# tonfengerqiguyisui/mapping-private

Hardware: AMD Instinct MI355X
Metric: Mvoxels/s C3-HLAC + detections/s sliding-box, 256^3 grid (higher is better)
Workload: dtype u8 x u8 -> u32 (exact integer C3-HLAC), f32 search

## Files before the change

mapping-private_amd/csrc/c3h_internal.h:

```cpp
#pragma once
#include <hip/hip_runtime.h>

#include <cstdint>
#include <cstdlib>
#include <string>
#include <mutex>
#include <vector>

#include "../../include/c3hlac_mi355x.h"

namespace c3h {

constexpr uint32_t kOcc = 1u << 24;
constexpr uint32_t kEmptyKey = 0xffffffffu;
constexpr int kBlock = 256;
constexpr int kTileMax = 16;

constexpr float kNorm0 = 1 / 255.0;
constexpr float kNorm1 = 1 / 65025.0;
constexpr float kNorm117_1 = 1 / 845325.0;
constexpr float kNorm117_1Bin = 1 / 13.0;

template <class T>
struct DevBuf {
  T* p = nullptr;
  size_t n = 0;
};

struct SearchLists {
  int rank = 0, M = 0;
  std::vector<double> score;
  std::vector<int32_t> x, y, z, mode;
// ... 207 lines not shown
  int atomic;
  const uint32_t* lut;
  float* feat;
  int32_t* exist;
  unsigned long long* acc64;
  const int16_t* axmap;
  int ar_s = 0, ar_oy = 0, ar_oz = 0;
  uint32_t ar_magic = 0;
  int32_t* work;
  int32_t* rows;
  uint32_t epoch;
  int zero_empty;
  int zero_feat;
  int64_t ntiles;
  long long* prof;
  int debug;
  uint32_t* dense = nullptr;
  _Float16* feat16 = nullptr;
  uint32_t* feat16_flag = nullptr;
  int f16s = 0;
  const uint32_t* vl_words = nullptr;
  const int32_t* vl_counts = nullptr;
  int vl_nseg = 0, vl_seg = 0, vl_count_stride = 0;
};

int64_t c3hlac_grid(const C3Launch& a);
hipError_t launch_c3hlac(const C3Launch& a, hipStream_t s);
hipError_t launch_colour_hist(const uint32_t* grid, int64_t nvox, unsigned long long* out, hipStream_t s);
hipError_t launch_offcell_delta(const int32_t* rec, int nrec, const C3Launch& l, int hist1, const int off[3],
                                const int sb[3], float inv_s, hipStream_t s);
hipError_t launch_c3_finalize(const unsigned long long* acc64, int64_t hist_num, int variant,
                              float* feat, int32_t* exist, int nframes, hipStream_t s);
struct NbrGrid {
  const float4* pts;
  int64_t n;
  float origin[3];
  float cell, inv_cell;
  int dim[3];
  const uint32_t* sorted;
  const uint32_t* cstart;
  const uint32_t* cend;
};
struct GrsdArgs {
  const float4* cent;
  int64_t nc;
  const int32_t* layout;
// ... 117 lines not shown
};
hipError_t launch_replay(const double* scores, const ReplayModes& modes, int M, int rank,
                         int r1, int r2, int r3, int clean, c3h_det* lists, c3h_det* out2,
                         hipStream_t s);
struct ReplayFrames {
  const double* scores;
  int64_t s_scores;
  ReplayModes modes;
  int M, nf, rank;
  int r1, r2, r3;
  int clean;
  c3h_det* lists;
  int64_t s_lists;
  c3h_det* outs[kMaxBatch];
};
bool replay_frames_ok(const ReplayModes& modes, int rank);
hipError_t launch_replay_frames(const ReplayFrames& a, hipStream_t s);

hipError_t launch_clean_lists(c3h_det* lists, int n, hipStream_t s);

struct TickParts {
  const C3Launch* occ = nullptr;
  const C3Launch* tile = nullptr;
  const SparseSearch* gate = nullptr;
  const SparseCompress* comp = nullptr;
  const SparseSearch* score = nullptr;
  DevBuf<long long>* prof = nullptr;
};
bool tick_ok(const C3Launch& l);
hipError_t launch_tick(const TickParts& p, hipStream_t s);
size_t c3hlac_lds_bytes(int tw_max, int list_max);
int64_t leaf_layout_blocks(int64_t nvox);

}

struct c3h_ctx {
  int device = 0;
  hipStream_t stream = nullptr;
  hipStream_t own_stream = nullptr;
  std::string err;

  c3h_ctx* parent = nullptr;
  std::vector<c3h_ctx*> lanes;
  std::vector<hipEvent_t> lane_ev;
  hipEvent_t fork_ev = nullptr;
  int nlanes = 3;
// ... 37 lines not shown
  bool vcent_valid = false;
  int64_t n_offcell = 0;
  c3h::DevBuf<uint32_t> scratch;
  c3h::DevBuf<uint32_t> tmp_u32;
  c3h::DevBuf<int32_t> tmp_i32;
  uint32_t* h_small = nullptr;
  c3h::VoxFrameRec* h_recs = nullptr;
  size_t h_recs_n = 0;
  bool table_valid = false;

  bool have_feat = false;
  c3h_extract_params last{};
  int64_t hist_num = 0;
  int32_t subdiv_b[3] = {0, 0, 0};
  int feat_dim = 0;
  c3h::DevBuf<float> feat;
  c3h::DevBuf<int32_t> exist;
  c3h::DevBuf<unsigned long long> acc64;
  c3h::DevBuf<int32_t> segs;
  c3h::DevBuf<int16_t> axmap;
  std::vector<int16_t> h_axmap;
  c3h::DevBuf<uint32_t> tileflags;
  c3h::DevBuf<int32_t> work;
  uint32_t tile_epoch = 0;
  int cap_h2d = 0;
  int64_t tf_stride = -1;
  int tf_frames = 0;
  int nframes_feat = 1;
  c3h::DevBuf<int32_t> rows;
  bool rows_valid = false;
  bool g_sparse = false;
  bool feat_sparse = false;
  c3h::DevBuf<long long> glist;
  c3h::DevBuf<float> gbox;
  c3h::DevBuf<uint32_t> gcnt;
  uint32_t search_epoch = 0;
  int gcnt_frames = 0;
  c3h::DevBuf<long long> prof;
  c3h::DevBuf<unsigned long long> chist;

  std::vector<int32_t> h_segs;
  c3h::DevBuf<uint32_t> lut;
  bool lut_ready = false;

  bool have_setup = false;
  int D = 0, F = 0, M = 0, r = 0, Dpad = 0;
// ... 31 lines not shown
  size_t h_dl_n = 0;
  c3h::DevBuf<c3h_det> d_lists;
  bool lists_host_valid = true;
  bool lists_dev_valid = false;
  int32_t last_range[3] = {0, 0, 0};

  c3h::Timer timer;

  bool capture = false;
  bool cap_c3_valid = false, cap_search_valid = false, cap_sparse_g = false, cap_argmax = false;
  c3h::C3Launch cap_c3{};
  c3h::SparseSearch cap_q{};
  c3h::SparseCompress cap_sc{};
  bool cap_replay = false;
  c3h::ReplayFrames cap_rp{};

  struct PipeBatch {
    c3h::C3Launch l;
    c3h::SparseSearch q;
    c3h::SparseCompress sc;
    int nf;
    int age;
    bool stamped = false;
    c3h_ctx* set = nullptr;
    std::vector<int64_t> layout;
    bool fix = false;
    c3h::PointFixup fx{};
    bool replay = false;
    c3h::ReplayFrames rp{};
  };
  struct PipeKey {
    int32_t div_b[3], min_b[3];
    float leaf;
    c3h_extract_params p;
    int32_t range[3], thr, rotate, batch, rank;
    uint64_t setup_version;
  };
  c3h::DevBuf<uint32_t> pb_grid, pb_wlist;
  c3h::DevBuf<int32_t> pb_part, pb_lim;
  c3h::DevBuf<c3h::VoxFlag> pb_flags;
  c3h::DevBuf<uint32_t> pb_bucket, pb_xcnt;
  c3h::DevBuf<uint32_t> dense_flag;
  c3h::DevBuf<c3h::VoxMoved> pb_moved;
  int64_t pb_cvox = 0;
  int pb_slots = 0;
  int pb_prev_nf = 0, pb_prev_total = 0;
// ... 20 lines not shown
```

mapping-private_amd/csrc/c3hlac_dev.h:

```cpp
#pragma once
#include <type_traits>

#include "c3h_internal.h"
#include "occ_sched.h"

namespace c3h {

constexpr int kArrStride = 196;
constexpr int kChunk = 128;
constexpr int kGroups = kChunk / 4;

__device__ __forceinline__ int bin981(int k, int c, int n) {
  return k <= 8 ? 6 + 78 * c + 9 * n + k : 60 + 78 * c + 4 * n + (k - 9);
}
__device__ __forceinline__ int tri6(int c, int n) { return 6 * c - c * (c - 1) / 2 + (n - c); }

__device__ __forceinline__ int bin_of(int type, int k, int n, int c) {
  if (k <= 12) return (type ? 495 : 0) + bin981(k, c, n);
  if (k == 13) {
    if (type == 0) return c <= n ? 474 + tri6(c, n) : -1;
    if (c <= 1 && n >= 2) return 969 + 4 * c + (n - 2);
    if ((c == 2 || c == 3) && n >= 4) return 977 + 2 * (c - 2) + (n - 4);
    return -1;
  }
// ... 63 lines not shown
    if (cur == -1) {
      const int old = atomicCAS(&s_set[h], -1, t);
      if (old == -1 || old == t) return;
    }
  }
  stamp_tile(t, epoch, flags, cnt, work);
}

struct OccArgs {
  const uint32_t* grid[kMaxBatch];
  int gx, gy, gz;
  const int16_t* axmap;
  int ns0, ns1;
  int ntiles;
  uint32_t epoch;
  uint32_t* tf;
  int32_t* work;
  int64_t s_tf, s_work;
  int contiguous;
  int steal_from = 0, steal_unit = 0, steal_units = 0, nframes = 0, steal_wgs = 0;
  int ar_s = 0, ar_oy = 0, ar_oz = 0;
  uint32_t ar_magic = 0;
  const uint32_t* dense = nullptr;
};

constexpr int kOccBitsMax = 1 << 18;
#ifndef C3H_OCC_PIPE
#define C3H_OCC_PIPE 0
#endif
#ifndef C3H_OCC_ARITH
#define C3H_OCC_ARITH 1
#endif
constexpr bool kOccArith = C3H_OCC_ARITH;
#ifndef C3H_OCC_PAIR
#define C3H_OCC_PAIR 1
#endif
#ifndef C3H_OCC_RING
#define C3H_OCC_RING 0
#endif
static_assert(kOccSchedBlock == kBlock, "occ_sched.h: threads per streaming workgroup");
constexpr bool kOccPipe = C3H_OCC_PIPE;
typedef unsigned int v4u __attribute__((ext_vector_type(4)));
constexpr int kAxLds = 3072;

__device__ __forceinline__ int block_excl_scan(int v, int* s_wsum, int* total) {
  const int lane = threadIdx.x & 63, wid = threadIdx.x >> 6;
// ... 112 lines not shown
    uint32_t mA = 0, mB = 0;
    bool cplx = false;
#pragma unroll
    for (int k = 0; k < 4; ++k) {
      if (tx0[k] < 0) continue;
      if (tA < 0 || tx0[k] == tA) {
        tA = tx0[k];
        mA |= 1u << k;
      } else if (tB < 0 || tx0[k] == tB) {
        tB = tx0[k];
        mB |= 1u << k;
      } else {
        cplx = true;
      }
    }
    const bool pair_ok = C3H_OCC_PAIR && __ballot(cplx) == 0ull;
    constexpr int kRow = kOccRowUnroll;
    constexpr int kChunkR = kBlock * kRow;
    const int lg = gx == 256 ? 8 : gx == 512 ? 9 : 10;
    const OccSched sc =
        occ_sched(n4, kRow, gdx, oa.contiguous, oa.steal_from, oa.steal_unit, oa.steal_units, oa.nframes);
    const int64_t nch = sc.nch, nstat = sc.nstat;
    uint4 w[kRow];
    auto chunk_of = [&](int64_t i) { return occ_chunk_of(sc, bx, i); };
    auto load_row = [&](uint64_t base, uint32_t voff, int j) {
      uint64_t bj = base + (uint64_t)j * (kBlock * 16);
      asm volatile("" : "+s"(bj));
      typedef const __attribute__((address_space(1))) char* gptr;
      const v4u t = __builtin_nontemporal_load(
          reinterpret_cast<const __attribute__((address_space(1))) v4u*>(reinterpret_cast<gptr>(bj) + voff));
      return make_uint4(t.x, t.y, t.z, t.w);
    };
    auto chunk_base = [&](int64_t c, uint32_t& voff) {
      uint64_t base = reinterpret_cast<uint64_t>(g4) + (uint64_t)c * (kChunkR * 16);
      voff = (uint32_t)tid * 16u;
      asm volatile("" : "+s"(base), "+v"(voff));
      return base;
    };
    auto load_any = [&](int64_t c) {
      uint32_t voff;
      if (occ_chunk_whole(sc, c)) {
        const uint64_t base = chunk_base(c, voff);
#pragma unroll
        for (int j = 0; j < kRow; ++j) w[j] = load_row(base, voff, j);
      } else {
        const uint64_t base = chunk_base(c, voff);
#pragma unroll
        for (int j = 0; j < kRow; ++j)
          w[j] = occ_wave_load_inside(sc, c, j, wv) ? load_row(base, voff, j) : make_uint4(0, 0, 0, 0);
      }
    };
    auto proc = [&](uint32_t row0) {
      int y = (int)(row0 % (uint32_t)gy), z = (int)(row0 / (uint32_t)gy);
#pragma unroll
      for (int j = 0; j < kRow; ++j) {
        const int yj = y, zjj = z;
        y += rpj;
        while (y >= gy) {
          y -= gy;
          ++z;
        }
        const uint32_t ws[4] = {w[j].x, w[j].y, w[j].z, w[j].w};
        if (__ballot((ws[0] | ws[1] | ws[2] | ws[3]) != 0u) == 0ull || zjj >= gz) continue;
        int a, b;
        if (oa.ar_s) {
          a = yj >= oa.ar_oy ? (int)__umulhi((uint32_t)(yj - oa.ar_oy), oa.ar_magic) : -1;
          b = zjj >= oa.ar_oz ? (int)__umulhi((uint32_t)(zjj - oa.ar_oz), oa.ar_magic) : -1;
        } else {
          a = __builtin_amdgcn_readfirstlane(my[yj]);
          b = __builtin_amdgcn_readfirstlane(mz[zjj]);
        }
        if (a < 0 || b < 0) continue;
        const int tyz = ns0 * (a + ns1 * b);
        if (pair_ok) {
          const uint32_t o = min(ws[0], 1u) | (min(ws[1], 1u) << 1) | (min(ws[2], 1u) << 2) | (min(ws[3], 1u) << 3);
          const int ta = tA + tyz, tb = tB + tyz;
          if (o & mA) atomicOr(&s_bits[ta >> 5], 1u << (ta & 31));
          if (o & mB) atomicOr(&s_bits[tb >> 5], 1u << (tb & 31));
          continue;
        }
#pragma unroll
        for (int k = 0; k < 4; ++k) {
          const int t = tx0[k] + tyz;
          if (ws[k] && tx0[k] >= 0 && t != last) {
            last = t;
            atomicOr(&s_bits[t >> 5], 1u << (t & 31));
          }
        }
      }
    };
#if C3H_OCC_RING
    const int64_t nfull = min(n4 / kChunkR, nstat);
    int64_t ri = 0;
    if (chunk_of(0) < nfull) {
#if C3H_OCC_RING == 2
      auto chunk_rsrc = [&](int64_t c) { return reinterpret_cast<const char*>(g4 + c * kChunkR); };
      auto ring_load = [&](const char* r, int j) {
        return __builtin_nontemporal_load(reinterpret_cast<const v4u*>(r + voff + j * kBlock * 16));
      };
#else
      auto chunk_rsrc = [&](int64_t c) {
        return __builtin_amdgcn_make_buffer_rsrc((void*)(g4 + c * kChunkR), (short)0, kChunkR * 16, 0x00020000);
      };
      auto ring_load = [&](__amdgpu_buffer_rsrc_t r, int j) {
        return __builtin_amdgcn_raw_buffer_load_b128(r, voff, j * kBlock * 16, 2);
      };
#endif
      int64_t cur = chunk_of(0);
      {
        const auto r = chunk_rsrc(cur);
#pragma unroll
        for (int j = 0; j < kRow; ++j) {
// ... 54 lines not shown
    if (kOccPipe && chunk_of(0) < nch) load_chunk(w, chunk_of(0) * kChunkR);
    for (int64_t i = 0; i < sc.per; ++i) {
#endif
      const int64_t cidx = chunk_of(i);
      if (cidx >= nstat) continue;
      const int64_t c0 = cidx * kChunkR;
      uint4 nx[kRow];
      if constexpr (kOccPipe) {
        const int64_t cn = chunk_of(i + 1);
        if (cn < nch) load_chunk(nx, cn * kChunkR);
      } else {
        load_any(cidx);
      }
      const uint32_t row0 = (uint32_t)(((uint64_t)c0 * 4 + (uint64_t)wv * 256) >> lg);
#ifdef C3H_OCC_NOPROC
      {
        uint32_t o = 0;
#pragma unroll
        for (int j = 0; j < kRow; ++j) o |= w[j].x | w[j].y | w[j].z | w[j].w;
        if (o == 0x12345678u) atomicOr(&s_bits[0], 1u);
        continue;
      }
#endif
      proc(row0);
      if constexpr (kOccPipe) {
#pragma unroll
        for (int j = 0; j < kRow; ++j) w[j] = nx[j];
      }
    }
    __syncthreads();
    occ_flush_bits(s_bits, nwords, s_list, s_wsum, epoch, flags, cnt, work);
    if (oa.steal_unit > 0) {
      uint32_t* pool = oa.tf;
      for (;;) {
        __syncthreads();
        if (tid == 0) s_wsum[15] = (int)atomicAdd(pool, 1u);
        __syncthreads();
        const int u = __builtin_amdgcn_readfirstlane(s_wsum[15]);
        if (u >= oa.steal_units) {
          if (tid == 0 && atomicAdd(oa.tf + 1, 1u) == (uint32_t)oa.steal_wgs - 1) {
            atomicExch(pool, 0u);
            atomicExch(oa.tf + 1, 0u);
          }
          break;
        }
        const OccUnit un = occ_unit(sc, u);
        const int fu = un.frame;
        for (int i = tid; i < nwords; i += kBlock) s_bits[i] = 0u;
        last = -1;
        g4 = reinterpret_cast<const uint4*>(oa.grid[fu]);
        __syncthreads();
        for (int64_t c = un.cb; c < un.ce; ++c) {
          load_any(c);
          proc((uint32_t)(((uint64_t)c * kChunkR * 4 + (uint64_t)wv * 256) >> lg));
        }
        __syncthreads();
        occ_flush_bits(s_bits, nwords, s_list, s_wsum, epoch, oa.tf + fu * oa.s_tf + 4,
                       oa.tf + fu * oa.s_tf + 2 + (epoch & 1), oa.work + fu * oa.s_work);
      }
    }
    return;
  }
  uint4 w[kOccBitsUnroll];
  int64_t c0 = bx * (int64_t)kChunk4;
  if (c0 < n4) load_chunk(w, c0);
  for (; c0 < n4; c0 += cstride) {
    uint4 nx[kOccBitsUnroll];
    if (kOccPipe && c0 + cstride < n4) load_chunk(nx, c0 + cstride);
    const uint32_t v0 = (uint32_t)((c0 + tid) << 2);
    const uint32_t row0 = v0 / (uint32_t)gx;
    int x = (int)(v0 - row0 * (uint32_t)gx);
    int y = (int)(row0 % (uint32_t)gy), z = (int)(row0 / (uint32_t)gy);
    int tyz[kOccBitsUnroll];
    int txj[kOccBitsUnroll];
#pragma unroll
    for (int j = 0; j < kOccBitsUnroll; ++j) {
      const int ty = my[y], tz = mz[min(z, gz - 1)];
// ... 65 lines not shown
  int tw_max, list_max;
  int thr_r, thr_g, thr_b;
  int variant, atomic;
  const uint32_t* lut;
  float* feat;
  int32_t* exist;
  unsigned long long* acc64;
  const uint32_t* flags;
  const int32_t* work;
  uint32_t* workcnt;
  int32_t* rows;
  uint32_t epoch;
  int ntiles;
  int zero_feat;
  int zblocks;
  long long* prof;
  int wave117;
  int mfma;
  int mf_pb;
  _Float16* feat16;
  uint32_t* feat16_flag;
  int f16s;
  int debug;
};

constexpr int kMaxLoads = 4;
constexpr int kSegLds = 64;
#ifndef C3H_TILE_PREFETCH
#define C3H_TILE_PREFETCH 0
#endif
static __device__ const uint4 kHaloZero16 = {0u, 0u, 0u, 0u};

struct HaloGeo {
  int y0, z0, ly, TY, q4, n, xs;
  bool vec;
};
__device__ __forceinline__ HaloGeo halo_geo(const KArgs& a, const int32_t* segs, int tile);

#define C3H_PROF(k, cond) \
  if (fprof && tid == 0 && (cond)) fprof[bx * 8 + (k)] = (long long)wall_clock64()

__device__ __forceinline__ HaloGeo halo_geo(const KArgs& a, const int32_t* segs, int tile) {
  const int ix = tile % a.ns0, iy = (tile / a.ns0) % a.ns1, iz = tile / (a.ns0 * a.ns1);
  const int32_t* sx = segs + 3 * ix;
  const int32_t* sy = segs + 3 * (a.seg_stride + iy);
  const int32_t* sz = segs + 3 * (2 * a.seg_stride + iz);
// ... 363 lines not shown
      float* row = ffeat + (int64_t)tj * a.variant;
      for (int c = lane; c < a.variant; c += 64) row[c] = 0.0f;
      if (lane == 0) fexist[tj] = 0;
    }
  }
}

struct W117Geom {
  int x0, lx, y0, ly, z0, lz;
  int64_t h;
};

__device__ __forceinline__ W117Geom w117_geom(const KArgs& a, const int32_t* segs, int tile) {
  const int ix = tile % a.ns0, iy = (tile / a.ns0) % a.ns1, iz = tile / (a.ns0 * a.ns1);
  const int32_t* sx = segs + 3 * ix;
  const int32_t* sy = segs + 3 * (a.seg_stride + iy);
  const int32_t* sz = segs + 3 * (2 * a.seg_stride + iz);
  W117Geom g;
  g.x0 = sx[0]; g.lx = sx[1]; g.y0 = sy[0]; g.ly = sy[1]; g.z0 = sz[0]; g.lz = sz[1];
  g.h = sx[2] + (int64_t)sy[2] * a.sbx + (int64_t)sz[2] * a.sbx * a.sby;
  return g;
}

__device__ __forceinline__ void w117_load_halo(const KArgs& a, const uint32_t* __restrict__ fgrid, const W117Geom& g,
                                               bool valid, int lane, uint32_t (&hv)[kW117HaloRegs]) {
  const int TX = g.lx + 2, TY = g.ly + 2, n = valid ? TX * TY * (g.lz + 1) : 0;
  int q = lane / TX, r = lane - (lane / TX) * TX;
  const int sq = 64 / TX, sr = 64 - sq * TX;
#pragma unroll
  for (int j = 0; j < kW117HaloRegs; ++j) {
    const int e = lane + 64 * j;
    const int yy = g.y0 - 1 + q % TY, zz = g.z0 - 1 + q / TY, xx = g.x0 - 1 + r;
    const bool in = e < n && (unsigned)xx < (unsigned)a.gx && (unsigned)yy < (unsigned)a.gy &&
                    (unsigned)zz < (unsigned)a.gz;
    const uint32_t v = fgrid[in ? ((int64_t)zz * a.gy + yy) * a.gx + xx : 0];
    hv[j] = in ? v : 0u;
    q += sq;
    r += sr;
    if (r >= TX) {
      r -= TX;
      ++q;
    }
  }
}

__device__ __forceinline__ void wave_lds_fence() { __asm__ volatile("s_waitcnt lgkmcnt(0)" ::: "memory"); }

typedef unsigned short w117_u16x2 __attribute__((ext_vector_type(2)));

__device__ __forceinline__ uint32_t w117_pk(uint32_t l) { return (l & 0xffu) | ((l & 0xff00u) << 8); }
__device__ __forceinline__ uint32_t w117_beta(bool bt) { return bt ? 1u : 0x10000u; }

__device__ __forceinline__ uint32_t udot2(uint32_t x, uint32_t y, uint32_t acc) {
  return __builtin_amdgcn_udot2(__builtin_bit_cast(w117_u16x2, x), __builtin_bit_cast(w117_u16x2, y), acc, false);
}

__device__ __forceinline__ void c3hlac_wave117_body(const KArgs& a, int bx, int fy_, int gdx, uint32_t* smem) {
  const int64_t fy = fy_;
// ... 20 lines not shown
  uint16_t* s_list = reinterpret_cast<uint16_t*>(s_halo + ((a.tw_max + 3) & ~3));
  uint32_t* s_ch = s_halo + ((a.tw_max + 3) & ~3) + (((a.list_max + 1) / 2 + 3) & ~3);
  uint16_t* s_ch16 = reinterpret_cast<uint16_t*>(s_ch);
  const int NW = (gdx - a.zblocks) * kW117Waves;
  int wi = (bx - a.zblocks) * kW117Waves + wave;
  int t_cur = wi < a.ntiles ? fwork[wi] : 0;
  int t_nxt = wi + NW < a.ntiles ? fwork[wi + NW] : 0;
  const int nwork = (int)fworkcnt[a.epoch & 1];
  s_lut[tid] = a.lut[tid];
  const bool segs_lds = a.seg_stride <= kSegLds;
  const int32_t* segs = segs_lds ? s_segs : a.segs;
  if (segs_lds)
    for (int e = tid; e < 9 * a.seg_stride; e += kBlock) s_segs[e] = a.segs[e];
  lds_barrier();
  C3H_PROF(1, true);
  if (wave >= kW117Waves || wi >= nwork) return;
  bool first = true;
  int X0, Y0, X1 = 0, Y1 = 0;
  w117_bin_channels(lane, X0, Y0);
  const bool has1 = lane + 64 < 117;
  if (has1) w117_bin_channels(lane + 64, X1, Y1);
  uint32_t hv[kW117HaloRegs];
  W117Geom g = w117_geom(a, segs, t_cur);
  w117_load_halo(a, fgrid, g, true, lane, hv);
  const int thr_r = a.thr_r, thr_g = a.thr_g, thr_b = a.thr_b;
  for (; wi < nwork; wi += NW) {
    const int TX = g.lx + 2, TY = g.ly + 2, TXY = TX * TY;
    const int nh = TXY * (g.lz + 1);
    int nlist = 0;
    {
      int q = lane / TX, r = lane - q * TX;
      int qy = q % TY, qz = q / TY;
      const int sq = 64 / TX, sr = 64 - sq * TX;
#pragma unroll
      for (int j = 0; j < kW117HaloRegs; ++j) {
        const int e = lane + 64 * j;
        if (e < nh) s_halo[e] = hv[j];
        const bool occ = e < nh && hv[j] != 0u && (unsigned)(r - 1) < (unsigned)g.lx &&
                         (unsigned)(qy - 1) < (unsigned)g.ly && qz >= 1;
        const unsigned long long m = __ballot(occ);
        if (occ) s_list[nlist + __popcll(m & ((1ull << lane) - 1))] = (uint16_t)e;
        nlist += __popcll(m);
        r += sr;
        qy += sq;
        if (r >= TX) {
          r -= TX;
          ++qy;
        }
        while (qy >= TY) {
          qy -= TY;
          ++qz;
        }
      }
    }
    const W117Geom gc = g;
    const bool more = wi + NW < nwork;
    const int t_after = wi + 2 * NW < a.ntiles ? fwork[wi + 2 * NW] : 0;
    if (more) {
      g = w117_geom(a, segs, t_nxt);
      w117_load_halo(a, fgrid, g, true, lane, hv);
    }
    t_nxt = t_after;
    wave_lds_fence();
    C3H_PROF(2, first);
    C3H_PROF(3, first);
    uint32_t acc0 = 0, acc1 = 0;
    for (int c0 = 0; c0 < nlist; c0 += 64) {
      uint32_t one = 0, cA[3] = {0, 0, 0}, cB[3] = {0, 0, 0}, cN[3] = {0, 0, 0}, cQ[3] = {0, 0, 0};
      if (c0 + lane < nlist) {
        const int ti = s_list[c0 + lane];
        uint32_t wn[13];
#pragma unroll
        for (int k = 0; k < 13; ++k) {
          const int rdx = k <= 8 ? k / 3 - 1 : (k <= 11 ? k - 10 : -1);
          const int rdy = k <= 8 ? k % 3 - 1 : (k <= 11 ? -1 : 0);
          const int rdz = k <= 8 ? -1 : 0;
          wn[k] = s_halo[ti + rdx + rdy * TX + rdz * TXY];
        }
        const uint32_t w = s_halo[ti];
        const uint32_t r = (w >> 16) & 0xffu, gg = (w >> 8) & 0xffu, b = w & 0xffu;
        one = 1;
        cA[0] = w117_pk(s_lut[r]);
        cA[1] = w117_pk(s_lut[gg]);
        cA[2] = w117_pk(s_lut[b]);
        cB[0] = w117_beta((int)r > thr_r);
// ... 88 lines not shown
```

mapping-private_amd/csrc/capi.hip:

```cpp
#include <algorithm>
#include <climits>
#include <cmath>
#include <cstdio>
#include <cstdlib>
#include <cstring>
#include <thread>

#include "c3h_internal.h"

using c3h::DevBuf;

namespace {

int fail(c3h_ctx* ctx, int code, const std::string& msg) {
  if (ctx) ctx->err = msg;
  return code;
}
int hip_fail(c3h_ctx* ctx, const char* what, hipError_t e) {
  return fail(ctx, C3H_ERR_HIP, std::string(what) + ": " + hipGetErrorString(e));
}

#define HIPCHK(expr)                                     \
  do {                                                   \
    hipError_t e_ = (expr);                              \
    if (e_ != hipSuccess) return hip_fail(ctx, #expr, e_); \
  } while (0)

template <class T>
int ensure(c3h_ctx* ctx, DevBuf<T>& b, size_t n) {
  if (n == 0) n = 1;
  if (b.n >= n) return C3H_OK;
// ... 684 lines not shown
  release(ctx->vosch_feat);
  release(ctx->vacc);
  release(ctx->vmg);
  release(ctx->vtpos);
  release(ctx->vlcnt);
  release(ctx->vlists);
  release(ctx->vcnt);
  release(ctx->vpart);
  release(ctx->vcounts);
  release(ctx->voffs);
  release(ctx->vcur);
  release(ctx->vbucket);
  release(ctx->vcent);
  release(ctx->voffcell);
  release(ctx->scratch);
  release(ctx->tmp_u32);
  release(ctx->tmp_i32);
  release(ctx->feat);
  release(ctx->exist);
  release(ctx->acc64);
  release(ctx->segs);
  release(ctx->axmap);
  release(ctx->tileflags);
  release(ctx->rows);
  release(ctx->work);
  release(ctx->glist);
  release(ctx->gbox);
  release(ctx->gcnt);
  release(ctx->lut);
  release(ctx->axis_pt);
  release(ctx->axis_pt16);
  release(ctx->axis_q);
  release(ctx->fmax);
  release(ctx->G);
  release(ctx->scores);
  release(ctx->qt);
  release(ctx->partials);
  release(ctx->d_lists);
  release(ctx->prof);
  release(ctx->chist);
  release(ctx->qt16);
  release(ctx->pb_grid);
  release(ctx->pb_wlist);
  release(ctx->pb_part);
  release(ctx->pb_lim);
  release(ctx->dense_flag);
// ... 663 lines not shown
        return -1;
      };
      const int oy = first(my, div[1]), oz = first(mz, div[2]);
      int S = 0;
      if (oy >= 0) {
        while (oy + S < div[1] && my[oy + S] == 0) ++S;
      }
      const uint32_t magic = S > 0 ? (uint32_t)(0x100000000ull / (uint64_t)S) + 1u : 0u;
      auto closed = [&](const int16_t* m, int n, int off) {
        if (off < 0) return false;
        for (int c = 0; c < n; ++c) {
          const int v = c >= off ? (int)(((uint64_t)(uint32_t)(c - off) * magic) >> 32) : -1;
          if (v != m[c]) return false;
        }
        return true;
      };
      const bool ok = S > 0 && oz >= 0 && closed(my, div[1], oy) && closed(mz, div[2], oz);
      l.ar_s = ok ? S : 0;
      l.ar_oy = oy;
      l.ar_oz = oz;
      l.ar_magic = magic;
    }
    ENSURE(ctx->work, (size_t)nf * ntiles);
    l.tf = ctx->tileflags.p;
    l.work = ctx->work.p;
    l.rows = nullptr;
    if (!atomic) {
      ENSURE(ctx->rows, (size_t)nf * hist_num);
      l.rows = ctx->rows.p;
    }
    ctx->rows_valid = !atomic;
    l.epoch = ctx->tile_epoch;
    l.zero_empty = (!atomic && all_covered) ? 1 : 0;
    l.zero_feat = 0;
    ctx->feat_sparse = l.zero_empty && !l.zero_feat;
    l.ntiles = ntiles;
    l.debug = 0;
    l.prof = nullptr;
    l.dense = nullptr;
    const bool from_list = kVoxListStamp && !ctx->capture && nf == 1 && ctx->table_valid &&
                           ctx->grid_ptr == ctx->grid.p && ctx->vargs.lists &&
                           (int64_t)ctx->vns * 16 < (int64_t)div[0] * div[1] * div[2];
    if (from_list) {
      const c3h::VoxArgs& va = ctx->vargs;
      l.vl_words = va.lists + (size_t)(2 + va.par) * va.lcap;
      l.vl_counts = va.part + (size_t)va.par * va.nblk_cap * c3h::vox_part_words() + c3h::kVoxPartNew;
// ... 652 lines not shown
}

struct PipeScope {
  c3h_ctx* ctx;
  hipStream_t saved[kPipeDepth - 1];
  explicit PipeScope(c3h_ctx* c) : ctx(c) {
    ctx->pipe_busy = true;
    for (int l = 0; l < kPipeDepth - 1 && l < (int)ctx->lanes.size(); ++l) {
      saved[l] = ctx->lanes[l]->stream;
      ctx->lanes[l]->stream = ctx->stream;
    }
  }
  ~PipeScope() {
    for (int l = 0; l < kPipeDepth - 1 && l < (int)ctx->lanes.size(); ++l) ctx->lanes[l]->stream = saved[l];
    ctx->pipe_busy = false;
  }
};

int pipe_tick(c3h_ctx* ctx, const c3h_ctx::PipeBatch* fresh) {
  c3h::TickParts tp;
  tp.prof = &ctx->prof;
  if (fresh && !fresh->stamped) tp.occ = &fresh->l;
  for (auto& b : ctx->pipe) {
    if (b.age == 1) tp.tile = &b.l;
    if (b.age == 2) {
      tp.gate = &b.q;
      tp.comp = &b.sc;
    }
    if (b.age == 3) tp.score = &b.q;
  }
  {
    Timed tm(ctx, 5, fresh ? fresh->nf : 0);
    hipError_t e = c3h::launch_tick(tp, ctx->stream);
    if (e != hipSuccess) return hip_fail(ctx, "launch_tick", e);
  }
  for (auto& b : ctx->pipe) {
    if (b.age == 3 && b.replay) {
      Timed tm(ctx, 4, b.nf);
      hipError_t e = c3h::launch_replay_frames(b.rp, ctx->stream);
      if (e != hipSuccess) return hip_fail(ctx, "launch_replay_frames", e);
    }
    if (b.age == 2 && b.set) b.set->scores_layout = b.layout;
    if (b.age == 1 && b.fix) {
      hipError_t e = c3h::launch_point_fixup(b.fx, ctx->stream);
      if (e != hipSuccess) return hip_fail(ctx, "launch_point_fixup", e);
    }
  }
  std::vector<c3h_ctx::PipeBatch> next;
  for (auto& b : ctx->pipe)
    if (b.age < 3) {
      next.push_back(b);
      next.back().age++;
    }
  if (fresh) {
    next.push_back(*fresh);
    next.back().age = 1;
  }
  ctx->pipe.swap(next);
  return C3H_OK;
}

int pipe_flush(c3h_ctx* ctx) {
  if (ctx->pipe.empty()) return C3H_OK;
  PipeScope scope(ctx);
  while (!ctx->pipe.empty()) {
    int rc = pipe_tick(ctx, nullptr);
    if (rc != C3H_OK) {
      ctx->pipe.clear();
      return rc;
    }
  }
  return C3H_OK;
}

int pipe_quiesce(c3h_ctx* ctx) {
  if (ctx->pipe_busy || ctx->pipe.empty()) return C3H_OK;
  return pipe_flush(ctx);
}

// ... 783 lines not shown
```

mapping-private_amd/csrc/occ_sched.h:

```cpp
#pragma once
#include <cstdint>

#if defined(__HIPCC__)
#define C3H_SCHED_HD __host__ __device__ inline
#else
#define C3H_SCHED_HD inline
#endif

namespace c3h {

constexpr int kOccSchedBlock = 256;

#ifndef C3H_OCC_UNROLL
#define C3H_OCC_UNROLL 16
#endif
#ifndef C3H_OCC_ROW_UNROLL
#define C3H_OCC_ROW_UNROLL 16
#endif
constexpr int kOccBitsUnroll = C3H_OCC_UNROLL;
constexpr int kOccRowUnroll = C3H_OCC_ROW_UNROLL;

C3H_SCHED_HD bool occ_rowwave(int gx, bool ax) { return ax && (gx & 255) == 0 && 1024 % gx == 0; }
C3H_SCHED_HD int occ_depth(bool rowwave) { return rowwave ? kOccRowUnroll : kOccBitsUnroll; }
C3H_SCHED_HD int64_t occ_nchunks(int64_t n4, int depth) {
// ... 35 lines not shown

C3H_SCHED_HD bool occ_chunk_whole(const OccSched& s, int64_t c) { return (c + 1) * s.chunk4 <= s.n4; }

C3H_SCHED_HD int64_t occ_word(const OccSched& s, int64_t c, int j, int tid) {
  return c * s.chunk4 + (int64_t)j * kOccSchedBlock + tid;
}

C3H_SCHED_HD bool occ_wave_load_inside(const OccSched& s, int64_t c, int j, int wave) {
  return occ_word(s, c, j, wave * 64) < s.n4;
}

struct OccUnit {
  int frame;
  int64_t cb, ce;
};
C3H_SCHED_HD OccUnit occ_unit(const OccSched& s, int u) {
  OccUnit r;
  r.frame = u % s.nframes;
  r.cb = s.nstat + (int64_t)(u / s.nframes) * s.steal_unit;
  r.ce = r.cb + s.steal_unit < s.nch ? r.cb + s.steal_unit : s.nch;
  return r;
}

struct OccSteal {
  int from, unit, units;
};
inline OccSteal occ_steal_plan(int64_t nch, int nframes, int div, int unit) {
  OccSteal p{0, 0, 0};
  if (div <= 0 || unit <= 0 || nch < 2 * (int64_t)div) return p;
  const int64_t tail = nch / div;
  p.from = (int)(nch - tail);
  p.unit = unit;
  p.units = (int)(nframes * ((tail + unit - 1) / unit));
  return p;
}

}
```

mapping-private_amd/csrc/pipeline.hip:

```cpp
#include <algorithm>
#include <climits>
#include <cstdio>
#include <cstdlib>
#include <cstring>
#include <vector>

#include "c3hlac_dev.h"
#include "search_dev.h"

namespace c3h {
namespace {

struct TickArgs {
  int n_score, n_cg, n_tile, n_occ;
  SparseSearch sq;
  int s_gx, s_groups;
  int s_mpp;
  SparseSearch gq;
  CompressRows cr;
  int g_ngate, g_ncomp;
  int comp_mfma;
  KArgs ka;
  int t_grid;
  OccArgs oa;
// ... 127 lines not shown
          fmin = std::min(fmin, (hi[f] - t0) * 0.01);
          fmax = std::max(fmax, (hi[f] - t0) * 0.01);
          wmax = std::max(wmax, (hi[f] - lo[f]) * 0.01);
        }
        fprintf(fp, " occ_frame_end[%.1f..%.1f within<=%.1f]", fmin, fmax, wmax);
        std::vector<double> ends;
        for (int b = b0; b < b0 + n[r]; ++b) ends.push_back((v[2 * b + 1] - t0) * 0.01);
        std::sort(ends.begin(), ends.end());
        fprintf(fp, " occ_end_p10/50/90[%.1f %.1f %.1f]", ends[ends.size() / 10], ends[ends.size() / 2],
                ends[ends.size() * 9 / 10]);
      }
    }
    b0 += n[r];
  }
  fprintf(fp, "\n");
  fclose(fp);
}

int env_int(const char* name, int dflt) {
  const char* v = diag_env(name);
  return v && *v ? atoi(v) : dflt;
}

}

bool tick_ok(const C3Launch& l) {
  const C3Args c = build_c3_args(l);
  return c.bits && c.ax && !l.atomic && l.prof == nullptr && l.debug == 0;
}

hipError_t launch_tick(const TickParts& p, hipStream_t s) {
  TickArgs t{};
  size_t lds = 16;
#ifndef C3H_TICK_ORDER_DEFAULT
#define C3H_TICK_ORDER_DEFAULT 0x2130
#endif
  t.order = p.occ ? C3H_TICK_ORDER_DEFAULT : 0x3210;
  if (const char* o = diag_env("C3H_TICK_ORDER"))
    if (strlen(o) == 4) {
      t.order = 0;
      for (int i = 0; i < 4; ++i) t.order |= (o[i] - '0') << (4 * i);
    }
  if (p.score) {
    const SparseSearch& a = *p.score;
    t.sq = a;
    t.s_gx = (int)std::max<int64_t>(1, std::min<int64_t>(sparse_score_blocks(a), env_int("C3H_TICK_SCORE", 16)));
// ... 21 lines not shown
    t.gq = a;
    t.cr = CompressRows{sc.feat, sc.PT, sc.fmax, sc.G, sc.rows, sc.nrows, sc.F, sc.D, sc.Dpad,
                        sc.fmax_len, sc.s_feat, sc.s_G, sc.s_rows, sc.s_nrows};
    t.g_ngate = (int)((a.pstart[a.nmodes] + kBlock - 1) / kBlock);
#ifndef C3H_TICK_COMP_MFMA
#define C3H_TICK_COMP_MFMA 1
#endif
    t.comp_mfma = env_int("C3H_TICK_COMP_MFMA", C3H_TICK_COMP_MFMA) && sc.Dpad <= 128 ? 1 : 0;
    if (t.comp_mfma) {
      t.g_ncomp = (int)std::max<int64_t>(1, std::min<int64_t>((sc.H + kCR - 1) / kCR, env_int("C3H_TICK_COMP", 16)));
      lds = std::max(lds, kTLds);
    } else {
      t.g_ncomp = (int)std::max<int64_t>(1, std::min<int64_t>((sc.H + kRR - 1) / kRR, env_int("C3H_TICK_COMP", 32)));
      lds = std::max(lds, compress_rows_lds_bytes(sc.Dpad));
    }
    t.n_cg = (t.g_ngate + t.g_ncomp) * a.nframes;
  }
  if (p.tile) {
    const C3Args c = build_c3_args(*p.tile);
    t.ka = c.ka;
    const int work = std::max(1, std::min(c.tgrid - c.ka.zblocks, env_int("C3H_TICK_TILE", 48)));
    t.ka.zblocks = std::min(c.ka.zblocks, env_int("C3H_TICK_ZERO", 8));
    t.t_grid = t.ka.zblocks + work;
    t.n_tile = t.t_grid * c.nframes;
    lds = std::max(lds, c.tile_lds);
  }
  if (p.occ) {
    const C3Args c = build_c3_args(*p.occ);
    t.oa = c.oa;
    t.o_grid = std::max(1, std::min(c.g1, env_int("C3H_TICK_OCC", std::max(1, 256 / std::max(1, c.nframes)))));
    t.n_occ = t.o_grid * c.nframes;
    lds = std::max(lds, c.occ_lds);
#ifndef C3H_TICK_STEAL_DIV
#define C3H_TICK_STEAL_DIV 16
#endif
#ifndef C3H_TICK_STEAL_UNIT
#define C3H_TICK_STEAL_UNIT 8
#endif
    const int64_t n4 = (int64_t)c.oa.gx * c.oa.gy * c.oa.gz / 4;
    const bool rowwave = occ_rowwave(c.oa.gx, c.ax);
    const int64_t nch = occ_nchunks(n4, occ_depth(rowwave));
    const int div = env_int("C3H_TICK_STEAL_DIV", C3H_TICK_STEAL_DIV);
    const int unit = env_int("C3H_TICK_STEAL_UNIT", C3H_TICK_STEAL_UNIT);
    const OccSteal st = rowwave ? occ_steal_plan(nch, c.nframes, div, unit) : OccSteal{0, 0, 0};
    if (st.unit > 0) {
      t.oa.steal_from = st.from;
      t.oa.steal_unit = st.unit;
      t.oa.steal_units = st.units;
      t.oa.nframes = c.nframes;
      t.oa.steal_wgs = t.n_occ;
    }
  }
  if (const char* m = diag_env("C3H_TICK_ROLES")) {
    const int mask = atoi(m);
    if (!(mask & 1)) t.n_score = 0;
    if (!(mask & 2)) t.n_cg = 0;
    if (!(mask & 4)) t.n_tile = 0;
    if (!(mask & 8)) t.n_occ = 0;
  }
  const int total = t.n_score + t.n_cg + t.n_tile + t.n_occ;
  if (total == 0) return hipSuccess;
#ifndef C3H_TICK_XCD
#define C3H_TICK_XCD 15
#endif
  t.xcd = 0;
  {
    const int nb[4] = {t.n_occ, t.n_tile, t.n_cg, t.n_score};
    const int per[4] = {t.o_grid, t.t_grid, t.g_ngate + t.g_ncomp, t.s_gx * t.s_groups};
    int base = 0;
    for (int i = 0; i < 4; ++i) {
      const int r = (t.order >> (4 * i)) & 15;
      if (nb[r] > 0 && per[r] > 0 && base % 8 == 0 && (nb[r] / per[r]) % 8 == 0) t.xcd |= 1 << r;
      base += nb[r];
    }
    t.xcd &= C3H_TICK_XCD;
  }
  if (diag_env("C3H_TICK_PROF") && p.prof) {
    DevBuf<long long>& b = *p.prof;
    if (b.n < (size_t)2 * total) {
      if (b.p) (void)hipFree(b.p);
      b.p = nullptr;
// ... 13 lines not shown
```

Baseline: 1.339 million.

## Record occupancy segment map in occ pass to skip empty halo loads in tile pass

The occupancy stage now writes a compact per-row bitmap (one bit per 16 voxels) from its existing ballots into a new segmap buffer. The next pipeline tick's wave117 tile kernel prefetches this map into LDS one tile ahead and masks halo loads for empty spans, so it can skip global reads of empty voxels. This adds extra map writes, an extra prefetch stage (lookahead grows from 2 to 3 tiles), and LDS traffic. It applies only under capture with row-wave geometry.

```diff
diff --git a/mapping-private_amd/csrc/c3h_internal.h b/mapping-private_amd/csrc/c3h_internal.h
--- a/mapping-private_amd/csrc/c3h_internal.h
+++ b/mapping-private_amd/csrc/c3h_internal.h
@@ -8,6 +8,7 @@
 #include <vector>
 
 #include "../../include/c3hlac_mi355x.h"
+#include "occ_sched.h"
 
 namespace c3h {
 
@@ -261,6 +262,8 @@
   const uint32_t* vl_words = nullptr;
   const int32_t* vl_counts = nullptr;
   int vl_nseg = 0, vl_seg = 0, vl_count_stride = 0;
+  occ_seg_t* segmap = nullptr;
+  int64_t s_segmap = 0;
 };
 
 int64_t c3hlac_grid(const C3Launch& a);
@@ -424,6 +427,7 @@
 struct TickParts {
   const C3Launch* occ = nullptr;
   const C3Launch* tile = nullptr;
+  bool tile_mapped = false;
   const SparseSearch* gate = nullptr;
   const SparseCompress* comp = nullptr;
   const SparseSearch* score = nullptr;
@@ -507,6 +511,7 @@
   std::vector<int16_t> h_axmap;
   c3h::DevBuf<uint32_t> tileflags;
   c3h::DevBuf<int32_t> work;
+  c3h::DevBuf<c3h::occ_seg_t> segmap;
   uint32_t tile_epoch = 0;
   int cap_h2d = 0;
   int64_t tf_stride = -1;
@@ -584,6 +589,7 @@
     int nf;
     int age;
     bool stamped = false;
+    bool mapped = false;
     c3h_ctx* set = nullptr;
     std::vector<int64_t> layout;
     bool fix = false;
diff --git a/mapping-private_amd/csrc/c3hlac_dev.h b/mapping-private_amd/csrc/c3hlac_dev.h
--- a/mapping-private_amd/csrc/c3hlac_dev.h
+++ b/mapping-private_amd/csrc/c3hlac_dev.h
@@ -109,6 +109,8 @@
   int ar_s = 0, ar_oy = 0, ar_oz = 0;
   uint32_t ar_magic = 0;
   const uint32_t* dense = nullptr;
+  occ_seg_t* segmap = nullptr;
+  int64_t s_segmap = 0;
 };
 
 constexpr int kOccBitsMax = 1 << 18;
@@ -267,6 +269,8 @@
         occ_sched(n4, kRow, gdx, oa.contiguous, oa.steal_from, oa.steal_unit, oa.steal_units, oa.nframes);
     const int64_t nch = sc.nch, nstat = sc.nstat;
     uint4 w[kRow];
+    static_assert(kRow <= 64, "one lane per row of a chunk holds the row's map entry");
+    occ_seg_t* smap = oa.segmap ? oa.segmap + f * oa.s_segmap : nullptr;
     auto chunk_of = [&](int64_t i) { return occ_chunk_of(sc, bx, i); };
     auto load_row = [&](uint64_t base, uint32_t voff, int j) {
       uint64_t bj = base + (uint64_t)j * (kBlock * 16);
@@ -295,8 +299,15 @@
           w[j] = occ_wave_load_inside(sc, c, j, wv) ? load_row(base, voff, j) : make_uint4(0, 0, 0, 0);
       }
     };
-    auto proc = [&](uint32_t row0) {
+    auto proc = [&](uint32_t row0, int64_t c) {
       int y = (int)(row0 % (uint32_t)gy), z = (int)(row0 / (uint32_t)gy);
+      uint32_t blo = 0, bhi = 0;
+      uint32_t lv = (uint32_t)tid & 63u;
+      asm volatile("" : "+v"(lv));
+      auto put_map = [&] {
+        if (smap && lv < (uint32_t)kRow)
+          smap[c * (kChunkR >> 6) + lv * (kBlock / 64) + wv] = occ_seg_make(((uint64_t)bhi << 32) | blo);
+      };
 #pragma unroll
       for (int j = 0; j < kRow; ++j) {
         const int yj = y, zjj = z;
@@ -306,7 +317,10 @@
           ++z;
         }
         const uint32_t ws[4] = {w[j].x, w[j].y, w[j].z, w[j].w};
-        if (__ballot((ws[0] | ws[1] | ws[2] | ws[3]) != 0u) == 0ull || zjj >= gz) continue;
+        const unsigned long long bal = __ballot((ws[0] | ws[1] | ws[2] | ws[3]) != 0u);
+        if (bal == 0ull || zjj >= gz) continue;
+        blo = lv == (uint32_t)j ? (uint32_t)bal : blo;
+        bhi = lv == (uint32_t)j ? (uint32_t)(bal >> 32) : bhi;
         int a, b;
         if (oa.ar_s) {
           a = yj >= oa.ar_oy ? (int)__umulhi((uint32_t)(yj - oa.ar_oy), oa.ar_magic) : -1;
@@ -333,6 +347,7 @@
           }
         }
       }
+      put_map();
     };
 #if C3H_OCC_RING
     const int64_t nfull = min(n4 / kChunkR, nstat);
@@ -433,7 +448,7 @@
         continue;
       }
 #endif
-      proc(row0);
+      proc(row0, cidx);
       if constexpr (kOccPipe) {
 #pragma unroll
         for (int j = 0; j < kRow; ++j) w[j] = nx[j];
@@ -460,10 +475,11 @@
         for (int i = tid; i < nwords; i += kBlock) s_bits[i] = 0u;
         last = -1;
         g4 = reinterpret_cast<const uint4*>(oa.grid[fu]);
+        if (smap) smap = oa.segmap + fu * oa.s_segmap;
         __syncthreads();
         for (int64_t c = un.cb; c < un.ce; ++c) {
           load_any(c);
-          proc((uint32_t)(((uint64_t)c * kChunkR * 4 + (uint64_t)wv * 256) >> lg));
+          proc((uint32_t)(((uint64_t)c * kChunkR * 4 + (uint64_t)wv * 256) >> lg), c);
         }
         __syncthreads();
         occ_flush_bits(s_bits, nwords, s_list, s_wsum, epoch, oa.tf + fu * oa.s_tf + 4,
@@ -575,6 +591,8 @@
   uint32_t* feat16_flag;
   int f16s;
   int debug;
+  const occ_seg_t* segmap = nullptr;
+  int64_t s_segmap = 0;
 };
 
 constexpr int kMaxLoads = 4;
@@ -984,18 +1002,63 @@
   return g;
 }
 
+constexpr int kW117MapRegs = 3;
+#ifndef C3H_W117_SKIP
+#define C3H_W117_SKIP 0
+#endif
+constexpr int kW117MapWords = kW117MapRegs;
+__host__ __device__ inline bool w117_map_fits(int lx, int ly, int lz) {
+  return (ly + 2) * (lz + 1) <= 64 * kW117MapRegs && lx + 2 <= 16;
+}
+__device__ __forceinline__ int w117_map_off(int xs, int gx) { return min(xs >> 5, (gx >> 5) - 2); }
+__device__ __forceinline__ int w117_map_sb(int xs, int gx) { return C3H_SEG_RAW ? 2 * w117_map_off(xs, gx) : (xs >> 8) << 4; }
+__device__ __forceinline__ void w117_load_map(const KArgs& a, const occ_seg_t* __restrict__ fmap, const W117Geom& g,
+                                              int lane, uint32_t (&me)[kW117MapWords]) {
+  const int TY = g.ly + 2, np = TY * (g.lz + 1);
+  const int rs = a.gx >> 8;
+  const int xs = max(g.x0 - 1, 0), xe = min(g.x0 + g.lx, a.gx - 1);
+#pragma unroll
+  for (int i = 0; i < kW117MapRegs; ++i) {
+    const int q = lane + 64 * i;
+    const int yy = g.y0 - 1 + q % TY, zz = g.z0 - 1 + q / TY;
+    const bool in = q < np && (unsigned)yy < (unsigned)a.gy && (unsigned)zz < (unsigned)a.gz;
+    const int64_t row = in ? ((int64_t)zz * a.gy + yy) * rs : 0;
+#if C3H_SEG_RAW
+    uint16_t two;
+    __builtin_memcpy(&two, reinterpret_cast<const uint8_t*>(fmap) + 8 * row + w117_map_off(xs, a.gx), 2);
+    me[i] = two;
+    (void)xe;
+#else
+    uint32_t e = fmap[row + (xs >> 8)];
+    if (rs > 1) e |= (uint32_t)fmap[row + (xe >> 8)] << 16;
+    me[i] = e;
+#endif
+  }
+}
+__device__ __forceinline__ void w117_put_map(uint32_t* s_map, int lane, const uint32_t (&me)[kW117MapWords]) {
+#pragma unroll
+  for (int i = 0; i < kW117MapRegs; ++i)
+    s_map[lane + 64 * i] = C3H_SEG_RAW ? occ_seg_fold32(me[i]) & 15u : me[i];
+  __asm__ volatile("s_waitcnt lgkmcnt(0)" ::: "memory");
+}
+
 __device__ __forceinline__ void w117_load_halo(const KArgs& a, const uint32_t* __restrict__ fgrid, const W117Geom& g,
-                                               bool valid, int lane, uint32_t (&hv)[kW117HaloRegs]) {
+                                               bool valid, int lane, uint32_t (&hv)[kW117HaloRegs],
+                                               const uint32_t* s_map = nullptr) {
   const int TX = g.lx + 2, TY = g.ly + 2, n = valid ? TX * TY * (g.lz + 1) : 0;
   int q = lane / TX, r = lane - (lane / TX) * TX;
   const int sq = 64 / TX, sr = 64 - sq * TX;
+  const int sb = w117_map_sb(max(g.x0 - 1, 0), a.gx);
 #pragma unroll
   for (int j = 0; j < kW117HaloRegs; ++j) {
     const int e = lane + 64 * j;
     const int yy = g.y0 - 1 + q % TY, zz = g.z0 - 1 + q / TY, xx = g.x0 - 1 + r;
-    const bool in = e < n && (unsigned)xx < (unsigned)a.gx && (unsigned)yy < (unsigned)a.gy &&
-                    (unsigned)zz < (unsigned)a.gz;
-    const uint32_t v = fgrid[in ? ((int64_t)zz * a.gy + yy) * a.gx + xx : 0];
+    bool in = e < n && (unsigned)xx < (unsigned)a.gx && (unsigned)yy < (unsigned)a.gy &&
+              (unsigned)zz < (unsigned)a.gz;
+    if (s_map) in = in && ((s_map[e < n ? q : 0] >> (((xx >> 4) - sb) & 31)) & 1u);
+    uint32_t v = 0u;
+    if (!(C3H_W117_SKIP && s_map) || __ballot(in) != 0ull)
+      v = fgrid[in ? ((int64_t)zz * a.gy + yy) * a.gx + xx : 0];
     hv[j] = in ? v : 0u;
     q += sq;
     r += sr;
@@ -1062,7 +1125,17 @@
   if (has1) w117_bin_channels(lane + 64, X1, Y1);
   uint32_t hv[kW117HaloRegs];
   W117Geom g = w117_geom(a, segs, t_cur);
-  w117_load_halo(a, fgrid, g, true, lane, hv);
+  const occ_seg_t* __restrict__ fmap = a.segmap ? a.segmap + fy * a.s_segmap : nullptr;
+  uint32_t* s_map = fmap ? s_ch : nullptr;
+  uint32_t me[kW117MapWords] = {};
+  int t_nx2 = 0;
+  if (fmap) {
+    t_nx2 = wi + 2 * NW < a.ntiles ? fwork[wi + 2 * NW] : 0;
+    w117_load_map(a, fmap, g, lane, me);
+    w117_put_map(s_map, lane, me);
+  }
+  w117_load_halo(a, fgrid, g, true, lane, hv, s_map);
+  if (fmap && wi + NW < nwork) w117_load_map(a, fmap, w117_geom(a, segs, t_nxt), lane, me);
   const int thr_r = a.thr_r, thr_g = a.thr_g, thr_b = a.thr_b;
   for (; wi < nwork; wi += NW) {
     const int TX = g.lx + 2, TY = g.ly + 2, TXY = TX * TY;
@@ -1095,12 +1168,20 @@
     }
     const W117Geom gc = g;
     const bool more = wi + NW < nwork;
-    const int t_after = wi + 2 * NW < a.ntiles ? fwork[wi + 2 * NW] : 0;
+    const int ahead = fmap ? 3 : 2;
+    const int t_after = wi + ahead * NW < a.ntiles ? fwork[wi + ahead * NW] : 0;
     if (more) {
       g = w117_geom(a, segs, t_nxt);
-      w117_load_halo(a, fgrid, g, true, lane, hv);
-    }
-    t_nxt = t_after;
+      if (fmap) w117_put_map(s_map, lane, me);
+      w117_load_halo(a, fgrid, g, true, lane, hv, s_map);
+      if (fmap && wi + 2 * NW < nwork) w117_load_map(a, fmap, w117_geom(a, segs, t_nx2), lane, me);
+    }
+    if (fmap) {
+      t_nxt = t_nx2;
+      t_nx2 = t_after;
+    } else {
+      t_nxt = t_after;
+    }
     wave_lds_fence();
     C3H_PROF(2, first);
     C3H_PROF(3, first);
diff --git a/mapping-private_amd/csrc/capi.hip b/mapping-private_amd/csrc/capi.hip
--- a/mapping-private_amd/csrc/capi.hip
+++ b/mapping-private_amd/csrc/capi.hip
@@ -7,6 +7,7 @@
 #include <thread>
 
 #include "c3h_internal.h"
+#include "occ_sched.h"
 
 using c3h::DevBuf;
 
@@ -737,6 +738,7 @@
   release(ctx->segs);
   release(ctx->axmap);
   release(ctx->tileflags);
+  release(ctx->segmap);
   release(ctx->rows);
   release(ctx->work);
   release(ctx->glist);
@@ -1446,6 +1448,11 @@
       l.ar_magic = magic;
     }
     ENSURE(ctx->work, (size_t)nf * ntiles);
+    if (ctx->capture && c3h::occ_rowwave(div[0], true)) {
+      l.s_segmap = c3h::occ_seg_entries((int64_t)div[0] * div[1] * div[2] / 4, c3h::kOccRowUnroll);
+      ENSURE(ctx->segmap, (size_t)nf * l.s_segmap);
+      l.segmap = ctx->segmap.p;
+    }
     l.tf = ctx->tileflags.p;
     l.work = ctx->work.p;
     l.rows = nullptr;
@@ -2144,7 +2151,10 @@
   tp.prof = &ctx->prof;
   if (fresh && !fresh->stamped) tp.occ = &fresh->l;
   for (auto& b : ctx->pipe) {
-    if (b.age == 1) tp.tile = &b.l;
+    if (b.age == 1) {
+      tp.tile = &b.l;
+      tp.tile_mapped = b.mapped;
+    }
     if (b.age == 2) {
       tp.gate = &b.q;
       tp.comp = &b.sc;
@@ -2177,6 +2187,7 @@
   if (fresh) {
     next.push_back(*fresh);
     next.back().age = 1;
+    next.back().mapped = tp.occ != nullptr;
   }
   ctx->pipe.swap(next);
   return C3H_OK;
diff --git a/mapping-private_amd/csrc/occ_sched.h b/mapping-private_amd/csrc/occ_sched.h
--- a/mapping-private_amd/csrc/occ_sched.h
+++ b/mapping-private_amd/csrc/occ_sched.h
@@ -81,6 +81,36 @@
   return r;
 }
 
+constexpr int kOccSpanVox = 256;
+C3H_SCHED_HD int64_t occ_seg_entry(int64_t voxel) { return voxel >> 8; }
+C3H_SCHED_HD int occ_seg_bit(int64_t voxel) { return (int)((voxel >> 4) & 15); }
+C3H_SCHED_HD int occ_chunk_spans(int depth) { return kOccSchedBlock / 64 * depth; }
+C3H_SCHED_HD int64_t occ_seg_entries(int64_t n4, int depth) { return occ_nchunks(n4, depth) * occ_chunk_spans(depth); }
+C3H_SCHED_HD int64_t occ_span_of(const OccSched& s, int64_t c, int j, int wave) {
+  return c * (s.chunk4 >> 6) + (int64_t)j * (kOccSchedBlock / 64) + wave;
+}
+C3H_SCHED_HD uint32_t occ_seg_fold32(uint32_t b) {
+  uint32_t y = (b | (b >> 1) | (b >> 2) | (b >> 3)) & 0x11111111u;
+  y = (y | (y >> 3)) & 0x03030303u;
+  y = (y | (y >> 6)) & 0x000F000Fu;
+  return (y | (y >> 12)) & 0xFFu;
+}
+C3H_SCHED_HD uint16_t occ_seg_fold(uint64_t ballot) {
+  return (uint16_t)(occ_seg_fold32((uint32_t)ballot) | (occ_seg_fold32((uint32_t)(ballot >> 32)) << 8));
+}
+#ifndef C3H_SEG_RAW
+#define C3H_SEG_RAW 0
+#endif
+#if C3H_SEG_RAW
+typedef uint64_t occ_seg_t;
+C3H_SCHED_HD occ_seg_t occ_seg_make(uint64_t ballot) { return ballot; }
+C3H_SCHED_HD bool occ_seg_test(occ_seg_t e, int64_t voxel) { return ((e >> (4 * occ_seg_bit(voxel))) & 15u) != 0; }
+#else
+typedef uint16_t occ_seg_t;
+C3H_SCHED_HD occ_seg_t occ_seg_make(uint64_t ballot) { return occ_seg_fold(ballot); }
+C3H_SCHED_HD bool occ_seg_test(occ_seg_t e, int64_t voxel) { return ((e >> occ_seg_bit(voxel)) & 1u) != 0; }
+#endif
+
 struct OccSteal {
   int from, unit, units;
 };
diff --git a/mapping-private_amd/csrc/pipeline.hip b/mapping-private_amd/csrc/pipeline.hip
--- a/mapping-private_amd/csrc/pipeline.hip
+++ b/mapping-private_amd/csrc/pipeline.hip
@@ -173,6 +173,11 @@
   return v && *v ? atoi(v) : dflt;
 }
 
+bool tick_segmap_ok(const C3Launch& l, const C3Args& c) {
+  return l.segmap && !C3H_OCC_RING && c.bits && occ_rowwave(l.gx, c.ax) && c.ka.wave117 &&
+         w117_map_fits(l.lmax[0], l.lmax[1], l.lmax[2]);
+}
+
 }
 
 bool tick_ok(const C3Launch& l) {
@@ -240,12 +245,20 @@
     const int work = std::max(1, std::min(c.tgrid - c.ka.zblocks, env_int("C3H_TICK_TILE", 48)));
     t.ka.zblocks = std::min(c.ka.zblocks, env_int("C3H_TICK_ZERO", 8));
     t.t_grid = t.ka.zblocks + work;
+    if (p.tile_mapped && tick_segmap_ok(*p.tile, c)) {
+      t.ka.segmap = p.tile->segmap;
+      t.ka.s_segmap = p.tile->s_segmap;
+    }
     t.n_tile = t.t_grid * c.nframes;
     lds = std::max(lds, c.tile_lds);
   }
   if (p.occ) {
     const C3Args c = build_c3_args(*p.occ);
     t.oa = c.oa;
+    if (tick_segmap_ok(*p.occ, c)) {
+      t.oa.segmap = p.occ->segmap;
+      t.oa.s_segmap = p.occ->s_segmap;
+    }
     t.o_grid = std::max(1, std::min(c.g1, env_int("C3H_TICK_OCC", std::max(1, 256 / std::max(1, c.nframes)))));
     t.n_occ = t.o_grid * c.nframes;
     lds = std::max(lds, c.occ_lds);
@@ -275,6 +288,7 @@
     if (!(mask & 2)) t.n_cg = 0;
     if (!(mask & 4)) t.n_tile = 0;
     if (!(mask & 8)) t.n_occ = 0;
+    if (!(mask & 8)) t.ka.segmap = nullptr;
   }
   const int total = t.n_score + t.n_cg + t.n_tile + t.n_occ;
   if (total == 0) return hipSuccess;
```

After: 1.357 million (median of 6 runs). 1.01x the previous value.
